# dylkot/cNMF

Measured on AMD Instinct MI355X. Metric: NMF restarts/sec (50000x2000xK5..13), higher is better.
Workload: dtype f32 (exact integer f16 plane x 2 f16 planes with per-row exponent, f32 accumulate)

## Files before the change

cnmf_amd/csrc/gemm_host.hip.h:

```cpp
#pragma once

#include "pass_plan.h"


template <int MTW, int WM, int WN, bool NN, int TBK = BK>
static hipError_t launch_gemm_t(hipStream_t st, const float* A, int lda, const float* B, int ldb,
                                float* C, int ldc, long long cstride, int KC, int Ktot, int J,
                                int nsplit)
{
    constexpr int MW = WM * MTW * 32, JW = WN * 32;
    const int Kper = round_up((Ktot + nsplit - 1) / nsplit, BK);
    dim3 grid((J + JW - 1) / JW, KC / MW, nsplit);
    constexpr size_t lds = gemm_lds_bytes<MTW, WM, WN, NN, TBK>();
    {
        if (hipError_t e_ = dyn_lds_optin((const void*)gemm_kernel<MTW, WM, WN, NN, TBK>, (int)lds)) return e_;
    }
    gemm_kernel<MTW, WM, WN, NN, TBK><<<grid, 256, lds, st>>>(A, lda, B, ldb, C, ldc, cstride, Kper,
                                                             Ktot, J);
    return hipGetLastError();
}

template <bool NN>
static hipError_t launch_gemm(hipStream_t st, int variant, const float* A, int lda, const float* B,
                              int ldb, float* C, int ldc, long long cstride, int KC, int Ktot,
// ... 192 lines not shown
    const int N = (int)ctx->N, G = (int)ctx->G, Np = ctx->N_pad, Gp = ctx->G_pad;
    const size_t pb = (size_t)Np * Gp * 2;
    const size_t fa = (size_t)(Np / G3C_JW) * ((Gp / 16 + 31) / 32) * sizeof(unsigned), fb = (size_t)(Gp / G3C_JW) * ((Np / 16 + 31) / 32) * sizeof(unsigned);
    DevPool pool;
    int* shA = pool.get<int>(Np);
    int* shB = pool.get<int>(Gp);
    POOL_TRY(ctx, pool);
    OwnedLocal<GeneralPlanesF> L;
    HIP_TRY(ctx, hipMalloc(&L.X2h, pb));
    HIP_TRY(ctx, hipMalloc(&L.X2m, pb));
    HIP_TRY(ctx, hipMalloc(&L.Xt2h, pb));
    HIP_TRY(ctx, hipMalloc(&L.Xt2m, pb));
    HIP_TRY(ctx, hipMalloc(&L.sA, (size_t)Np * sizeof(float)));
    HIP_TRY(ctx, hipMalloc(&L.sB, (size_t)Gp * sizeof(float)));
    HIP_TRY(ctx, hipMalloc(&L.onesA, fa));
    HIP_TRY(ctx, hipMalloc(&L.onesB, fb));
    HIP_TRY(ctx, hipMemsetAsync(L.onesA, 0xff, fa, st));
    HIP_TRY(ctx, hipMemsetAsync(L.onesB, 0xff, fb, st));
    x2h_rowshift_kernel<<<(Np + 3) / 4, 256, 0, st>>>(ctx->X, Gp, N, G, 0, Np, shA, L.sA);
    x2h_rowshift_kernel<<<(Gp + 255) / 256, 256, 0, st>>>(ctx->X, Gp, N, G, 1, Gp, shB, L.sB);
    const long long total = (long long)Np * (Gp / 16);
    x2h_planes_kernel<<<(unsigned)((total + 255) / 256), 256, 0, st>>>(ctx->X, Gp, N, G, Np, Gp, G3C_JW, shA,
                                                                        (unsigned short*)L.X2h, (unsigned short*)L.X2m);
    x2h_planes_transpose_kernel<<<dim3(Np / 16, (Gp + 255) / 256), 256, 0, st>>>(ctx->X, Gp, N, G, Gp, Np, G3C_JW, shB,
                                                                                (unsigned short*)L.Xt2h, (unsigned short*)L.Xt2m);
    HIP_TRY(ctx, hipGetLastError());
    HIP_TRY(ctx, hipStreamSynchronize(st));
    ctx->x2.take(L);
    return CNMF_OK;
}

static hipError_t launch_gemm3c(hipStream_t st, const unsigned char* A3, const unsigned char* B1,
                                const unsigned char* Bhi, const unsigned int* hiflag, int Kb,
                                float* C, int ldc, long long cstride, int KC, int Jpad, int nsplit)
{
    {
        if (hipError_t e_ = dyn_lds_optin((const void*)gemm3c_kernel, g3c_lds_bytes(true))) return e_;
    }
    const int kb_per = (Kb + nsplit - 1) / nsplit;
    dim3 grid(Jpad / G3C_JW, KC / G3_MW, (Kb + kb_per - 1) / kb_per);
    gemm3c_kernel<<<grid, 512, g3c_lds_bytes(Bhi != nullptr), st>>>(A3, B1, Bhi, hiflag, Kb, C, ldc, cstride, kb_per);
    return hipGetLastError();
}

static hipError_t launch_gemm3c_streamk(hipStream_t st, const StreamK3& sk, const unsigned char* A3,
                                        const unsigned char* B1, const unsigned char* Bhi,
                                        const unsigned int* hiflag, float* C0, float* C1, float* C2, int ldc)
{
    {
        if (hipError_t e_ = dyn_lds_optin((const void*)gemm3c_streamk_kernel, g3c_lds_bytes(true))) return e_;
    }
    gemm3c_streamk_kernel<<<sk.P, 512, g3c_lds_bytes(Bhi != nullptr), st>>>(A3, B1, Bhi, hiflag, sk.Kb, C0, C1, C2, ldc,
                                                                            sk.MG, sk.T);
    return hipGetLastError();
}


struct G2Launch {
    const unsigned char* A2 = nullptr;
    const float* rscale = nullptr;
    XOperand x{};
    int Kb = 0;
    float* C[3] = {nullptr, nullptr, nullptr};
    int ldc = 0;
    unsigned long long livemask = ~0ull;
    long long cstride = 0; int KC = 0, Jpad = 0, nsplit = 1;
    const StreamK3* sk = nullptr;
    const CdKnobs* kn = nullptr;
};
using G2Fn = hipError_t (*)(hipStream_t, const G2Launch&);
struct G2Entry { G2Form form; G2Fn fn; };

template <int NSUB, bool HI, int VAR = 0, bool PART = false, bool GEN = false>
static hipError_t launch_gemm2h_t(hipStream_t st, const G2Launch& g)
{
    constexpr int lds = g2_lds_bytes(NSUB, HI);
    {
        if (hipError_t e_ = dyn_lds_optin((const void*)gemm2h_kernel<NSUB, HI, VAR, PART, GEN>, lds)) return e_;
    }
    int kb_per = (g.Kb + g.nsplit - 1) / g.nsplit;
    kb_per = ((kb_per + NSUB - 1) / NSUB) * NSUB;
    dim3 grid(g.Jpad / G3C_JW, g.KC / G3_MW, (g.Kb + kb_per - 1) / kb_per);
    gemm2h_kernel<NSUB, HI, VAR, PART, GEN><<<grid, 512, lds, st>>>(g.A2, g.x.plane, HI ? g.x.hi : nullptr, HI ? g.x.flags : nullptr, g.rscale,
                                                                   g.Kb, g.C[0], g.ldc, g.cstride, kb_per, g.x.colscale,
                                                                   PART ? g.livemask : ~0ull);
    return hipGetLastError();
}

template <int NSUB, bool HI, int VAR = 0, bool NTB = true, bool PART = false, bool GEN = false>
static hipError_t launch_gemm2h_streamk_t(hipStream_t st, const G2Launch& g)
{
    constexpr int lds = g2_lds_bytes(NSUB, HI);
    {
        if (hipError_t e_ = dyn_lds_optin((const void*)gemm2h_streamk_kernel<NSUB, HI, VAR, NTB, PART, GEN>, lds)) return e_;
    }
    const int xmap = g2_xmap(G2Form{true, NSUB, HI, VAR, NTB, PART, GEN}, g.kn->g2_xmap);
    gemm2h_streamk_kernel<NSUB, HI, VAR, NTB, PART, GEN><<<g.sk->P, 512, lds, st>>>(g.A2, g.x.plane, HI ? g.x.hi : nullptr,
                                                                                    HI ? g.x.flags : nullptr, g.rscale, g.Kb, g.C[0], g.C[1],
                                                                                    g.C[2], g.ldc, g.sk->MG, g.sk->T, xmap, g.x.colscale,
                                                                                    PART ? g.livemask : ~0ull);
    return hipGetLastError();
}

template <int NSUB, bool HI, int VAR, bool PART, bool GEN>
static constexpr G2Entry g2_ksplit() { return {G2Form{true, NSUB, HI, VAR, false, PART, GEN}, launch_gemm2h_t<NSUB, HI, VAR, PART, GEN>}; }
template <int NSUB, bool HI, int VAR, bool NTB, bool PART, bool GEN>
static constexpr G2Entry g2_streamk() { return {G2Form{true, NSUB, HI, VAR, NTB, PART, GEN}, launch_gemm2h_streamk_t<NSUB, HI, VAR, NTB, PART, GEN>}; }

static constexpr G2Entry G2_KSPLIT[] = {
    g2_ksplit<1, true, 0, false, true>(),  g2_ksplit<1, true, 0, true, true>(),  g2_ksplit<1, true, 4, false, true>(),
    g2_ksplit<1, true, 4, true, true>(),   g2_ksplit<1, true, 0, false, false>(), g2_ksplit<1, true, 0, true, false>(),
    g2_ksplit<2, false, 4, false, false>(), g2_ksplit<2, false, 4, true, false>(), g2_ksplit<1, false, 4, false, false>()};
static constexpr G2Entry G2_STREAMK[] = {
    g2_streamk<1, true, 0, false, true, true>(),   g2_streamk<1, true, 0, false, false, true>(),  g2_streamk<1, true, 0, true, false, true>(),
    g2_streamk<1, true, 4, false, true, true>(),   g2_streamk<1, true, 4, false, false, true>(),  g2_streamk<1, true, 4, true, false, true>(),
    g2_streamk<1, true, 0, false, true, false>(),  g2_streamk<1, true, 0, false, false, false>(), g2_streamk<1, true, 0, true, false, false>(),
    g2_streamk<2, false, 4, false, true, false>(), g2_streamk<2, false, 4, false, false, false>(), g2_streamk<2, false, 4, true, false, false>(),
    g2_streamk<1, false, 4, false, false, false>(), g2_streamk<1, false, 4, true, false, false>()};

static G2Form g2_form_of(const G2Launch& g, int KC, bool shared)
{
    const unsigned long long full = g2_full_mask(KC);
    return g2_form(g.x.hi != nullptr, g.x.colscale != nullptr, g.kn->g2_gen4, g.kn->g2_gvar, gemm2h_nsub(false, g.Kb, g.kn->g2_nsub),
                   (g.livemask & full) != full, shared);
}

static hipError_t launch_gemm2h(hipStream_t st, const G2Launch& g)
{
    G2Form f = g2_form_of(g, g.KC, false);
    f.NTB = false;
    for (const G2Entry& e : G2_KSPLIT) if (e.form == f) return e.fn(st, g);
    return hipErrorInvalidValue;
}

static hipError_t launch_gemm2h_streamk(hipStream_t st, const G2Launch& g)
{
    const G2Form f = g2_form_of(g, g.sk->MG * G3_MW, g.sk->MG > 1);
    for (const G2Entry& e : G2_STREAMK) if (e.form == f) return e.fn(st, g);
    return hipErrorInvalidValue;
}

static hipError_t launch_split2h(hipStream_t st, const float* src, int ld, int rows, int K, unsigned char* dst, int TR,
                                 const double* kscale, const float* rmax_part, int parts, float* inv_scale)
{
    if (split2h_wide(K)) {
        dim3 grid(split2h_col_groups(K, rows), rows / 16);
        split2h_tiled_kernel<16, 16><<<grid, 256, 0, st>>>(src, ld, K, TR, (unsigned short*)dst, kscale, rmax_part, parts, inv_scale);
    } else {
        dim3 grid(split2h_col_groups(K, rows), rows / 64);
        split2h_tiled_kernel<64, 4><<<grid, 256, 0, st>>>(src, ld, K, TR, (unsigned short*)dst, kscale, rmax_part, parts, inv_scale);
    }
    return hipGetLastError();
}

static hipError_t launch_rowmax_part(hipStream_t st, const float* V, int ld, int L, int rows, int span,
                                     const double* kscale, int parts, float* rmax_part)
{
    dim3 grid(parts, rows / 4);
    rowmax_part_kernel<<<grid, 256, 0, st>>>(V, ld, L, span, kscale, parts, rmax_part);
    return hipGetLastError();
}

static int ensure_counts(cnmf_ctx* ctx)
{
    const int fmt = ctx->knobs.gemm3 == 4 ? 4 : 3;
    if (ctx->counts.state == 1 && ctx->counts.fmt != fmt) {
        hipStreamSynchronize(ctx->stream);
        ctx->counts.release();
    }
    if (ctx->counts.state != 0) return CNMF_OK;
    auto absent = [ctx] { ctx->counts.state = -1; return CNMF_OK; };
    const int N = (int)ctx->N, G = (int)ctx->G;
    if (ctx->N_pad % G3C_JW || ctx->G_pad % G3C_JW || ctx->knobs.no_counts || !ctx->count_detect) return absent();
    hipStream_t st = ctx->stream;
    const int chunks = (N + CNT_ROWS - 1) / CNT_ROWS;
    DevPool pool;
    float* part = pool.get<float>((size_t)chunks * G);
    float* vmin = pool.get<float>(G);
    unsigned* fail = pool.get<unsigned>(G, true, st);
    float* unit = pool.get<float>(G);
    double* psx = pool.get<double>((size_t)chunks * G);
    double* psn = pool.get<double>((size_t)chunks * G);
// ... 91 lines not shown
```

cnmf_amd/csrc/kernels_gemm2h.hip.h:

```cpp
#pragma once
#include <hip/hip_runtime.h>
#include "kernels_gemm3.hip.h"

namespace cnmf {

typedef _Float16 f16x8 __attribute__((ext_vector_type(8)));
typedef float f32x4_g __attribute__((ext_vector_type(4)));
#ifdef CNMF_G2_LDS_STORE
constexpr bool G2_LDS_STORE = true;
#else
constexpr bool G2_LDS_STORE = false;
#endif

constexpr int G2_ROWB = 64;
constexpr int G2_A = G3_MW * G2_ROWB;
constexpr int G2_B = G3C_JW * 32;
constexpr float G2_COUNT_BASE = 2048.0f;

constexpr int g2_imgs(int nsub) { return nsub == 1 ? 4 : 3; }
constexpr int g2_img_bytes(int nsub, bool with_hi) { return nsub * (G2_A + (with_hi ? 2 : 1) * G2_B); }
constexpr int g2_lds_bytes(int nsub, bool with_hi) { return g2_imgs(nsub) * g2_img_bytes(nsub, with_hi); }

__device__ __forceinline__ unsigned short f16_bits(float x)
{
    const _Float16 h = (_Float16)x;
    return __builtin_bit_cast(unsigned short, h);
}
__device__ __forceinline__ float f16_to_f32(unsigned short b) { return (float)__builtin_bit_cast(_Float16, b); }

__device__ __forceinline__ int g2_row_shift(float mx)
{
    if (!(mx > 0.f)) return 0;
    int e;
    frexpf(mx, &e);
    const int s = 15 - e;
    return s > 120 ? 120 : (s < -110 ? -110 : s);
}

__device__ __forceinline__ void split2h(float y, unsigned short& h, unsigned short& m)
{
    h = f16_bits(y);
    m = f16_bits(y - f16_to_f32(h));
}

struct SplitFused { const int* shift_in; int* shift_out; };
template <int TROWS, int TKB>
__device__ __forceinline__ void split2h_tiled_body(const float* __restrict__ src, int ld, int K, int TR,
                                                   unsigned short* __restrict__ dst, const double* __restrict__ kscale,
                                                   const float* __restrict__ rmax_part, int parts,
                                                   float* __restrict__ inv_scale, int bx, int nbx, int by,
                                                   unsigned short* tile_, float* red_, SplitFused fu = SplitFused{nullptr, nullptr})
{
    static_assert(TROWS * TKB == 256, "tile = 256 (row, block) pairs");
    constexpr int NQ = 256 / TROWS;
    constexpr int KQ = TKB * 4;
    constexpr int RPP = 256 / KQ;
    unsigned short (*tile)[TROWS][32] = reinterpret_cast<unsigned short (*)[TROWS][32]>(tile_);
    float (*red)[TROWS] = reinterpret_cast<float (*)[TROWS]>(red_);
    const int t = threadIdx.x;
    const int r0 = by * TROWS;
    const int kq = t % KQ, rr = t / KQ;
    const int ntiles = K / (16 * TKB);
    const bool fused = fu.shift_in != nullptr;
    float4 v[4];
    if (!fused) {
        const int k0 = bx * 16 * TKB;
#pragma unroll
        for (int i = 0; i < 4; ++i)
            v[i] = *reinterpret_cast<const float4*>(src + (size_t)(r0 + rr + RPP * i) * ld + k0 + kq * 4);
    }
    {
        const int row = t % TROWS, qt = t / TROWS;
        float mx = 0.f;
        for (int p0 = qt; p0 < parts; p0 += 8 * NQ) {
            float v[8];
#pragma unroll
            for (int j = 0; j < 8; ++j) v[j] = (p0 + j * NQ < parts) ? rmax_part[(size_t)(r0 + row) * parts + p0 + j * NQ] : 0.f;
#pragma unroll
            for (int j = 0; j < 8; ++j) mx = fmaxf(mx, v[j]);
        }
        red[qt][row] = mx;
    }
    __syncthreads();
    int sh[4];
    bool redo = false;
#pragma unroll
    for (int i = 0; i < 4; ++i) {
        const int row = rr + RPP * i;
        float mx = 0.f;
#pragma unroll
        for (int q = 0; q < NQ; ++q) mx = fmaxf(mx, red[q][row]);
        sh[i] = g2_row_shift(mx);
        if (fused) {
            const int su = fu.shift_in[r0 + row];
            const float ymax = ldexpf(mx, su);
            const bool ok = !(mx > 0.f) || (ymax < 60000.0f && ymax >= 1024.0f);
            const bool keep = !(mx > 0.f) || (ymax < 46340.0f && ymax >= 8192.0f);
            if (bx == 0 && kq == 0) fu.shift_out[r0 + row] = (ok && keep) ? su : sh[i];
            if (ok) sh[i] = su; else redo = true;
        }
        if (bx == 0 && kq == 0) inv_scale[r0 + row] = ldexpf(1.0f, -sh[i]);
    }
    if (fused) {
        if (!__syncthreads_or(redo ? 1 : 0)) return;
// ... 164 lines not shown
{
    if (!transpose) {
        const int row = blockIdx.x * 4 + (threadIdx.x >> 6), lane = threadIdx.x & 63;
        if (row >= rows_pad) return;
        float mx = 0.f;
        if (row < N) for (int g = lane; g < G; g += 64) mx = fmaxf(mx, X[(size_t)row * ld + g]);
#pragma unroll
        for (int o = 32; o > 0; o >>= 1) mx = fmaxf(mx, __shfl_xor(mx, o, 64));
        if (lane == 0) { const int s = g2_row_shift(mx); shift[row] = s; inv_scale[row] = ldexpf(1.0f, -s); }
    } else {
        const int g = blockIdx.x * 256 + threadIdx.x;
        if (g >= rows_pad) return;
        float mx = 0.f;
        if (g < G) for (int r = 0; r < N; ++r) mx = fmaxf(mx, X[(size_t)r * ld + g]);
        const int s = g2_row_shift(mx);
        shift[g] = s; inv_scale[g] = ldexpf(1.0f, -s);
    }
}

__global__ __launch_bounds__(256) void x2h_planes_kernel(const float* __restrict__ X, int ld, int N, int G, int rows_pad,
                                                         int K, int TR, const int* __restrict__ shift,
                                                         unsigned short* __restrict__ dst_h, unsigned short* __restrict__ dst_m)
{
    const long long t = (long long)blockIdx.x * 256 + threadIdx.x;
    const int Kb = K / 16;
    if (t >= (long long)rows_pad * Kb) return;
    const int row = (int)(t / Kb), kb = (int)(t % Kb);
    const int s = shift[row];
    unsigned short ph[16], pm[16];
#pragma unroll
    for (int i = 0; i < 16; ++i) {
        const int g = kb * 16 + i;
        const float x = (row < N && g < G) ? X[(size_t)row * ld + g] : 0.f;
        split2h(ldexpf(x, s), ph[i], pm[i]);
    }
    const size_t blk = (size_t)(row / TR) * Kb + kb;
    store_plane_row_swz(dst_h + (blk * TR + (row % TR)) * 16, ph, row % TR);
    store_plane_row_swz(dst_m + (blk * TR + (row % TR)) * 16, pm, row % TR);
}

__global__ __launch_bounds__(256) void x2h_planes_transpose_kernel(const float* __restrict__ X, int ld, int N, int G,
                                                                   int rows_pad, int K, int TR,
                                                                   const int* __restrict__ shift,
                                                                   unsigned short* __restrict__ dst_h,
                                                                   unsigned short* __restrict__ dst_m)
{
    const int j = blockIdx.y * 256 + threadIdx.x;
    const int kb = blockIdx.x;
    if (j >= rows_pad) return;
    const int Kb = K / 16;
    const int s = shift[j];
    unsigned short ph[16], pm[16];
#pragma unroll
    for (int i = 0; i < 16; ++i) {
        const int c = kb * 16 + i;
        const float x = (j < G && c < N) ? X[(size_t)c * ld + j] : 0.f;
        split2h(ldexpf(x, s), ph[i], pm[i]);
    }
    const size_t blk = (size_t)(j / TR) * Kb + kb;
    store_plane_row_swz(dst_h + (blk * TR + (j % TR)) * 16, ph, j % TR);
    store_plane_row_swz(dst_m + (blk * TR + (j % TR)) * 16, pm, j % TR);
}

__global__ __launch_bounds__(256) void count_max_base_kernel(const float* __restrict__ X, int ld, int N, int G,
                                                             const float* __restrict__ unit, float base,
                                                             unsigned* __restrict__ any_big)
{
    const int g = blockIdx.x * 256 + threadIdx.x;
    if (g >= G) return;
    const float u = unit[g];
    if (u <= 0.f) return;
    const int r0 = blockIdx.y * 256, r1 = min(N, r0 + 256);
    bool big = false;
    for (int r = r0; r < r1; ++r) big |= rintf(X[(size_t)r * ld + g] / u) > base;
    if (big) atomicOr(any_big, 1u);
}

struct G2NoEpi { static constexpr bool enabled = false; };
template <int NSUB, bool HI, int VAR = 0, bool NTB = true, bool PART = false, bool GEN = false, class EPI = G2NoEpi>
__device__ __forceinline__ void gemm2h_segment(const unsigned char* __restrict__ A2, const unsigned char* __restrict__ B1,
                                               const unsigned char* __restrict__ Bhi,
                                               const unsigned int* __restrict__ hiflag,
                                               const float* __restrict__ rscale,
                                               int Kb, float* __restrict__ C, int ldc, int m0, int j0, int kb0,
                                               int nkb, unsigned char* smem, const float* __restrict__ cscale = nullptr,
                                               unsigned live = 0xffu, const EPI* epi = nullptr, bool whole_tile = false)
{
    constexpr int IMGS = g2_imgs(NSUB);
    constexpr int IMG = g2_img_bytes(NSUB, HI);
    constexpr int OFF_B = NSUB * G2_A;
    constexpr int OFF_H = OFF_B + NSUB * G2_B;
    constexpr int NA = NSUB * 2, NB = NSUB;
    constexpr int NDMA = NA + NB;
    const int tid = threadIdx.x;
    const int lane = tid & 63, wave = tid >> 6;
    const int grp = wave >> 2, wn = wave & 3;
    const int li = lane & 31, h = lane >> 5;
    const int nst = nkb / NSUB;
    const unsigned lv = PART ? (unsigned)__builtin_amdgcn_readfirstlane((int)((live >> (grp * 4)) & 0xfu)) : 0xfu;
#define G2_LIVE(m_) (!PART || ((lv >> (m_)) & 1u))

    const size_t jblk = ((size_t)(j0 / G3C_JW) * Kb + kb0);
    const unsigned char* abase = A2 + ((size_t)(m0 / G3_MW) * Kb + kb0) * G2_A + tid * 16;
    const unsigned char* bbase = B1 + jblk * G2_B + tid * 16;
    const unsigned char* hbase = HI ? Bhi + jblk * G2_B + tid * 16 : nullptr;
    unsigned int fw[5] = {0u, 0u, 0u, 0u, 0u};
    if (HI) {
        const int KW = (Kb + 31) >> 5, w0 = kb0 >> 5;
        const unsigned int* fr = hiflag + (size_t)(j0 / G3C_JW) * KW;
#pragma unroll
        for (int w = 0; w < 5; ++w)
            fw[w] = (nkb > 129) ? 0xFFFFFFFFu : ((w0 + w < KW) ? __builtin_amdgcn_readfirstlane(fr[w0 + w]) : 0u);
    }
    const int fbit0 = kb0 & 31;

    f32x16_3 acc[4][2];
#pragma unroll
    for (int m = 0; m < 4; ++m)
#pragma unroll
        for (int n = 0; n < 2; ++n)
#pragma unroll
            for (int r = 0; r < 16; ++r) acc[m][n][r] = 0.f;

    const int a_row = (grp * 128 + li) * G2_ROWB;
    const int a_s0 = ((0 + h) ^ ((li >> 2) & 3)) * 16, a_s1 = ((2 + h) ^ ((li >> 2) & 3)) * 16;
    const int b_off = OFF_B + (wn * 64 + li) * 32 + (h ^ ((li >> 3) & 1)) * 16;

#define G2_BLKFLAG(b_) (HI && ((fw[(fbit0 + (b_)) >> 5 > 4 ? 4 : (fbit0 + (b_)) >> 5] >> ((fbit0 + (b_)) & 31)) & 1u))
#define G2_ISSUE(s_)                                                                               \
    {                                                                                              \
        unsigned char* d_ = smem + ((s_) % IMGS) * IMG + wave * 1024;                              \
        const unsigned char* a_ = abase + (size_t)(s_) * (NSUB * G2_A);                            \
        _Pragma("unroll") for (int i = 0; i < NA; ++i)                                             \
            __builtin_amdgcn_global_load_lds(G3_AS1(a_ + i * 8192), G3_AS3(d_ + i * 8192), 16, 0, 0); \
                                        \
        _Pragma("unroll") for (int i = 0; i < NB; ++i)                                             \
            __builtin_amdgcn_global_load_lds(G3_AS1(bbase + (size_t)(s_) * (NSUB * G2_B) + i * 8192), \
                                             G3_AS3(d_ + OFF_B + i * 8192), 16, 0, NTB ? 2 : 0);   \
        if (HI) {                                                                                  \
            _Pragma("unroll") for (int i = 0; i < NB; ++i)                                         \
                if (G2_BLKFLAG((s_) * NSUB + i))                                                   \
                    __builtin_amdgcn_global_load_lds(G3_AS1(hbase + (size_t)(s_) * (NSUB * G2_B) + i * 8192), \
                                                     G3_AS3(d_ + OFF_H + i * 8192), 16, 0, NTB ? 2 : 0); \
        }                                                                                          \
    }
#define G2_FRAG(ptr_) __builtin_bit_cast(f16x8, *reinterpret_cast<const u32x4*>(ptr_))
#define G2_READ(s_)                                                                                \
    {                                                                                              \
        const unsigned char* bb = smem + ((s_) % IMGS) * IMG;                                      \
        _Pragma("unroll") for (int u = 0; u < NSUB; ++u) {                                         \
            _Pragma("unroll") for (int n = 0; n < 2; ++n) bq[u][n] = G2_FRAG(bb + b_off + u * G2_B + n * 32 * 32); \
            if (HI) { _Pragma("unroll") for (int n = 0; n < 2; ++n)                                \
                          bh[u][n] = G2_FRAG(bb + b_off + NSUB * G2_B + u * G2_B + n * 32 * 32); } \
            _Pragma("unroll") for (int m = 0; m < 4; ++m) {                                        \
                aq[u][m][0] = G2_FRAG(bb + u * G2_A + a_row + m * 32 * G2_ROWB + a_s0);            \
                aq[u][m][1] = G2_FRAG(bb + u * G2_A + a_row + m * 32 * G2_ROWB + a_s1);            \
            }                                                                                      \
        }                                                                                          \
        __builtin_amdgcn_sched_barrier(0);                                                         \
    }
#define G2_MFMA(b_, u_, m_, q_)                                                                    \
    if (G2_LIVE(m_)) {                                                                             \
    acc[m_][0] = __builtin_amdgcn_mfma_f32_32x32x16_f16(aq[u_][m_][q_], b_[u_][0], acc[m_][0], 0, 0, 0); \
    acc[m_][1] = __builtin_amdgcn_mfma_f32_32x32x16_f16(aq[u_][m_][q_], b_[u_][1], acc[m_][1], 0, 0, 0); }
#define G2_MFMA4(b_, u_, ma_, mb_)                                                                 \
    G2_MFMA(b_, u_, ma_, 1) G2_MFMA(b_, u_, mb_, 1) G2_MFMA(b_, u_, ma_, 0) G2_MFMA(b_, u_, mb_, 0)
#define G2_MFMA2H(b_, u_, ma_, mb_) G2_MFMA(b_, u_, ma_, 0) G2_MFMA(b_, u_, mb_, 0)
#define G2_HALF(ma_, mb_)                                                                          \
    _Pragma("unroll") for (int u = 0; u < NSUB; ++u) {                                             \
        G2_MFMA4(bq, u, ma_, mb_)                                                                  \
        if (HI) { if (hi_blk[u]) { if constexpr (GEN) { G2_MFMA2H(bh, u, ma_, mb_) } else { G2_MFMA4(bh, u, ma_, mb_) } } } \
    }
#define G2_WAIT_AHEAD(cnt_)                                                                        \
    {                                                                                              \
        if constexpr ((cnt_) * NDMA == 0) G3_WAIT_VM(0);                                           \
        else if constexpr ((cnt_) * NDMA == 3) G3_WAIT_VM(3);                                      \
        else if constexpr ((cnt_) * NDMA == 6) G3_WAIT_VM(6);                                      \
        else if constexpr ((cnt_) * NDMA == 12) G3_WAIT_VM(12);                                    \
        else G3_WAIT_VM(0);                                                                        \
    }

    f16x8 bq[NSUB][2], bh[NSUB][2], aq[NSUB][4][2];
    constexpr int AHEAD = IMGS - 1;
    constexpr bool SPREAD = VAR >= 1 && NSUB == 2 && !HI;
    constexpr bool SPREADG = VAR >= 1 && NSUB == 1 && ((HI && GEN) || !HI);
    constexpr bool PRIO = false;
    constexpr bool NOMFMA = VAR == 2, NODMA = VAR == 3 || VAR == 6 || VAR == 7, SPLITRD = VAR >= 4;
    static_assert(VAR != 1 && VAR != 5, "instruction streams 1 and 5 were retired");
    constexpr bool NOREAD = VAR == 6 || VAR == 7;
    constexpr bool NOBAR = VAR == 7;
    G3_WAIT_VM(0);
    G2_ISSUE(0)
    if (nst > 1) G2_ISSUE(1)
    if (AHEAD > 2 && nst > 2) G2_ISSUE(2)
    if (AHEAD > 2 && nst > 2) G2_WAIT_AHEAD(2) else if (nst > 1) G2_WAIT_AHEAD(1) else G2_WAIT_AHEAD(0)
    if (grp == 1) G3_RAW_BARRIER()
    if constexpr (SPREADG) {
        static_assert(!SPREADG || (IMGS == 4 && NA == 2 && NB == 1), "one-block spread stream: four images, pieces A0 A1 B (Bhi)");
#define G2G_PIECE(s_, i_)                                                                          \
        {                                                                                          \
            unsigned char* d_ = smem + ((s_) % IMGS) * IMG + wave * 1024;                          \
            if ((i_) < NA)                                                                         \
                __builtin_amdgcn_global_load_lds(G3_AS1(abase + (size_t)(s_) * G2_A + (i_) * 8192), \
                                                 G3_AS3(d_ + (i_) * 8192), 16, 0, 0);              \
            else if ((i_) == NA)                                                                   \
                __builtin_amdgcn_global_load_lds(G3_AS1(bbase + (size_t)(s_) * G2_B), G3_AS3(d_ + OFF_B), 16, 0, NTB ? 2 : 0); \
            else if constexpr (HI)                                                                 \
                __builtin_amdgcn_global_load_lds(G3_AS1(hbase + (size_t)(s_) * G2_B), G3_AS3(d_ + OFF_H), 16, 0, NTB ? 2 : 0); \
            __builtin_amdgcn_sched_barrier(0);                                                     \
        }
#define G2G_READ_A(s_)                                                                             \
        {                                                                                          \
            const unsigned char* bb = smem + ((s_) % IMGS) * IMG;                                  \
            _Pragma("unroll") for (int n = 0; n < 2; ++n) bq[0][n] = G2_FRAG(bb + b_off + n * 32 * 32); \
            _Pragma("unroll") for (int m = 0; m < 2; ++m) {                                        \
                aq[0][m][1] = G2_FRAG(bb + a_row + m * 32 * G2_ROWB + a_s1);                       \
                aq[0][m][0] = G2_FRAG(bb + a_row + m * 32 * G2_ROWB + a_s0);                       \
            }                                                                                      \
            if constexpr (HI) { _Pragma("unroll") for (int n = 0; n < 2; ++n) bh[0][n] = G2_FRAG(bb + b_off + G2_B + n * 32 * 32); } \
            __builtin_amdgcn_sched_barrier(0);                                                     \
        }
#define G2G_READ_B(s_)                                                                             \
        {                                                                                          \
            const unsigned char* bb = smem + ((s_) % IMGS) * IMG;                                  \
            _Pragma("unroll") for (int m = 2; m < 4; ++m) {                                        \
                aq[0][m][1] = G2_FRAG(bb + a_row + m * 32 * G2_ROWB + a_s1);                       \
                aq[0][m][0] = G2_FRAG(bb + a_row + m * 32 * G2_ROWB + a_s0);                       \
            }                                                                                      \
            __builtin_amdgcn_sched_barrier(0);                                                     \
        }
#define G2G_STEP(MORE_)                                                                            \
        {                                                                                          \
            G3_RAW_BARRIER()                                         \
            G2G_READ_A(s)                                                                          \
            G2_MFMA(bq, 0, 0, 1) G2_MFMA(bq, 0, 1, 1)                                              \
            if (MORE_) G2G_PIECE(s + AHEAD, 0)                                                     \
            G2_MFMA(bq, 0, 0, 0) G2_MFMA(bq, 0, 1, 0)                                              \
            G2G_READ_B(s)                                                                          \
            if (MORE_) G2G_PIECE(s + AHEAD, 1)                                                     \
            if constexpr (HI) { G2_MFMA(bh, 0, 0, 0) G2_MFMA(bh, 0, 1, 0) }                        \
            asm volatile("s_waitcnt lgkmcnt(0)" ::: "memory");                                     \
             \
            if (s + 1 < nst) { if (MORE_) { if constexpr (HI) G3_WAIT_VM(6); else G3_WAIT_VM(5); } else G3_WAIT_VM(0); } \
            G3_RAW_BARRIER()                                                              \
            G2_MFMA(bq, 0, 2, 1) G2_MFMA(bq, 0, 3, 1)                                              \
            if (MORE_) G2G_PIECE(s + AHEAD, 2)                                                     \
            G2_MFMA(bq, 0, 2, 0) G2_MFMA(bq, 0, 3, 0)                                              \
            if constexpr (HI) { if (MORE_) G2G_PIECE(s + AHEAD, 3)                                 \
                                G2_MFMA(bh, 0, 2, 0) G2_MFMA(bh, 0, 3, 0) }                        \
        }
        {
            int s = 0;
            const int n_main = nst - AHEAD;
            for (; s < n_main; ++s) G2G_STEP(true)
            for (; s < nst; ++s) G2G_STEP(false)
        }
#undef G2G_STEP
#undef G2G_READ_B
#undef G2G_READ_A
#undef G2G_PIECE
    } else if constexpr (!SPREAD) {
        for (int s = 0; s < nst; ++s) {
            bool hi_blk[NSUB];
#pragma unroll
            for (int u = 0; u < NSUB; ++u) hi_blk[u] = G2_BLKFLAG(s * NSUB + u);
            G3_RAW_BARRIER()
            if (s + AHEAD < nst) G2_ISSUE(s + AHEAD)
            G2_READ(s)
            if (PRIO) __builtin_amdgcn_s_setprio(1);
            G2_HALF(0, 1)
            if (PRIO) __builtin_amdgcn_s_setprio(0);
            asm volatile("s_waitcnt lgkmcnt(0)" ::: "memory");
            if (s + 1 < nst) {
                if (AHEAD > 2 && s + 3 < nst) G2_WAIT_AHEAD(2) else if (s + 2 < nst) G2_WAIT_AHEAD(1) else G2_WAIT_AHEAD(0)
// ... 12 lines not shown
                                                 G3_AS3(d_ + (i_) * 8192), 16, 0, 0);              \
            else                                                                                   \
                __builtin_amdgcn_global_load_lds(G3_AS1(bbase + (size_t)(s_) * (NSUB * G2_B) + ((i_) - NA) * 8192), \
                                                 G3_AS3(d_ + OFF_B + ((i_) - NA) * 8192), 16, 0, NTB ? 2 : 0); \
            __builtin_amdgcn_sched_barrier(0);                                                     \
        }
#define G2_MF(u_, m_, q_)                                                                          \
        if constexpr (NOMFMA) { asm volatile("" :: "v"(aq[u_][m_][q_]), "v"(bq[u_][0]), "v"(bq[u_][1])); }        \
        else { G2_MFMA(bq, u_, m_, q_) }
#define G2_READ_A(s_)                                                                              \
    {                                                                                              \
        const unsigned char* bb = smem + ((s_) % IMGS) * IMG;                                      \
        _Pragma("unroll") for (int u = 0; u < NSUB; ++u) {                                         \
            _Pragma("unroll") for (int n = 0; n < 2; ++n) bq[u][n] = G2_FRAG(bb + b_off + u * G2_B + n * 32 * 32); \
            _Pragma("unroll") for (int m = 0; m < 2; ++m) {                                        \
                aq[u][m][1] = G2_FRAG(bb + u * G2_A + a_row + m * 32 * G2_ROWB + a_s1);            \
                aq[u][m][0] = G2_FRAG(bb + u * G2_A + a_row + m * 32 * G2_ROWB + a_s0);            \
            }                                                                                      \
        }                                                                                          \
        __builtin_amdgcn_sched_barrier(0);                                                         \
    }
#define G2_READ_B(s_)                                                                              \
    {                                                                                              \
        const unsigned char* bb = smem + ((s_) % IMGS) * IMG;                                      \
        _Pragma("unroll") for (int u = 0; u < NSUB; ++u)                                           \
            _Pragma("unroll") for (int m = 2; m < 4; ++m) {                                        \
                aq[u][m][1] = G2_FRAG(bb + u * G2_A + a_row + m * 32 * G2_ROWB + a_s1);            \
                aq[u][m][0] = G2_FRAG(bb + u * G2_A + a_row + m * 32 * G2_ROWB + a_s0);            \
            }                                                                                      \
        __builtin_amdgcn_sched_barrier(0);                                                         \
    }
#define G2_STEP(MORE_)                                                                             \
        {                                                                                          \
            if constexpr (!NOBAR) G3_RAW_BARRIER()                                        \
            if constexpr (NOREAD) { if (s == 0) { G2_READ(s) } }                                   \
            else if constexpr (SPLITRD) { G2_READ_A(s) } else { G2_READ(s) }                       \
            G2_MF(0, 0, 1) G2_MF(0, 1, 1)                                                          \
            if (MORE_) G2_PIECE(s + AHEAD, 0)                                                      \
            G2_MF(0, 0, 0) G2_MF(0, 1, 0)                                                          \
            if constexpr (SPLITRD && !NOREAD) { G2_READ_B(s) }                                     \
            if (MORE_) G2_PIECE(s + AHEAD, 1)                                                      \
            G2_MF(1, 0, 1) G2_MF(1, 1, 1)                                                          \
            if (MORE_) G2_PIECE(s + AHEAD, 2)                                                      \
            G2_MF(1, 0, 0) G2_MF(1, 1, 0)                                                          \
            asm volatile("s_waitcnt lgkmcnt(0)" ::: "memory");                                     \
             \
            if (s + 1 < nst) { if (MORE_) G3_WAIT_VM(3); else G3_WAIT_VM(0); }                     \
            if constexpr (!NOBAR) G3_RAW_BARRIER()                                        \
            G2_MF(0, 2, 1) G2_MF(0, 3, 1)                                                          \
            if (MORE_) G2_PIECE(s + AHEAD, 3)                                                      \
            G2_MF(0, 2, 0) G2_MF(0, 3, 0)                                                          \
            if (MORE_) G2_PIECE(s + AHEAD, 4)                                                      \
            G2_MF(1, 2, 1) G2_MF(1, 3, 1)                                                          \
            if (MORE_) G2_PIECE(s + AHEAD, 5)                                                      \
            G2_MF(1, 2, 0) G2_MF(1, 3, 0)                                                          \
        }
        {
            int s = 0;
            const int n_main = NODMA ? 0 : nst - AHEAD;
            for (; s < n_main; ++s) G2_STEP(true)
            for (; s < nst; ++s) G2_STEP(false)
        }
#undef G2_STEP
#undef G2_READ_B
#undef G2_READ_A
#undef G2_MF
#undef G2_PIECE
    }
    if (grp == 0) G3_RAW_BARRIER()
#undef G2_WAIT_AHEAD
#undef G2_HALF
#undef G2_MFMA2H
#undef G2_MFMA4
#undef G2_MFMA
#undef G2_READ
#undef G2_FRAG
#undef G2_ISSUE
#undef G2_BLKFLAG

    if constexpr (EPI::enabled) {
        if (whole_tile && epi->on) { (*epi)(acc, rscale, C, ldc, m0, j0, smem); return; }
    }
    if (C == nullptr) return;
    const int j = j0 + wn * 64 + li;
    const float cs[2] = {(HI && cscale) ? cscale[j] : 1.0f, (HI && cscale) ? cscale[j + 32] : 1.0f};
    if constexpr (!PART && G2_LDS_STORE && g2_lds_bytes(NSUB, HI) >= 8 * 16384) {
        float* tw = reinterpret_cast<float*>(smem) + wave * 4096;
#pragma unroll
        for (int mp = 0; mp < 2; ++mp) {
#pragma unroll
            for (int mm = 0; mm < 2; ++mm) {
                const int m = 2 * mp + mm;
#pragma unroll
                for (int n = 0; n < 2; ++n)
#pragma unroll
                    for (int r = 0; r < 16; ++r) {
                        const int rl = 4 * h + (r & 3) + 8 * (r >> 2);
                        tw[(mm * 32 + rl) * 64 + n * 32 + li] = (acc[m][n][r] * rscale[m0 + grp * 128 + m * 32 + rl]) * cs[n];
                    }
            }
            __builtin_amdgcn_wave_barrier();
#pragma unroll
            for (int i = 0; i < 16; ++i) {
                const int c = 4 * i + (lane >> 4);
                const f32x4_g v = *reinterpret_cast<const f32x4_g*>(tw + c * 64 + 4 * (lane & 15));
                *reinterpret_cast<f32x4_g*>(C + (size_t)(m0 + grp * 128 + mp * 64 + c) * ldc + j0 + wn * 64 + 4 * (lane & 15)) = v;
            }
            __builtin_amdgcn_wave_barrier();
        }
    } else {
#pragma unroll
    for (int m = 0; m < 4; ++m) {
        if (!G2_LIVE(m)) continue;
        const int cbase = m0 + grp * 128 + m * 32 + 4 * h;
#pragma unroll
        for (int n = 0; n < 2; ++n)
#pragma unroll
            for (int r = 0; r < 16; ++r) {
                const int row = cbase + (r & 3) + 8 * (r >> 2);
                C[(size_t)row * ldc + j + n * 32] = (acc[m][n][r] * rscale[row]) * cs[n];
            }
    }
    }
#undef G2_LIVE
}

template <int NSUB, bool HI, int VAR = 0, bool PART = false, bool GEN = false>
__global__ __launch_bounds__(512) void gemm2h_kernel(const unsigned char* __restrict__ A2,
                                                     const unsigned char* __restrict__ B1,
                                                     const unsigned char* __restrict__ Bhi,
                                                     const unsigned int* __restrict__ hiflag,
                                                     const float* __restrict__ rscale, int Kb,
                                                     float* __restrict__ C, int ldc, long long c_split_stride,
                                                     int kb_per, const float* __restrict__ cscale = nullptr,
                                                     unsigned long long livemask = ~0ull)
{
    extern __shared__ __attribute__((aligned(16))) unsigned char smem3[];
    int jt = blockIdx.x, mg = blockIdx.y, z = blockIdx.z;
    if ((gridDim.z & 7) == 0) {
        const int L = blockIdx.x + (int)gridDim.x * (blockIdx.y + (int)gridDim.y * blockIdx.z);
        const int xcd = L & 7, idx = L >> 3;
        jt = idx % (int)gridDim.x;
        mg = (idx / (int)gridDim.x) % (int)gridDim.y;
        z = xcd + 8 * (idx / (int)(gridDim.x * gridDim.y));
    }
    const int kb0 = z * kb_per;
    const int nkb = min(kb_per, Kb - kb0);
    gemm2h_segment<NSUB, HI, VAR, true, PART, GEN>(A2, B1, Bhi, hiflag, rscale, Kb, C ? C + (size_t)z * c_split_stride : nullptr, ldc, mg * G3_MW,
                                              jt * G3C_JW, kb0, nkb, smem3, cscale, (unsigned)((livemask >> (8 * mg)) & 0xffu));
}

template <int NSUB, bool HI, int VAR = 0, bool NTB = true, bool PART = false, bool GEN = false, class EPI = G2NoEpi>
__global__ __launch_bounds__(512) void gemm2h_streamk_kernel(const unsigned char* __restrict__ A2,
                                                             const unsigned char* __restrict__ B1,
                                                             const unsigned char* __restrict__ Bhi,
                                                             const unsigned int* __restrict__ hiflag,
                                                             const float* __restrict__ rscale, int Kb,
                                                             float* __restrict__ C0, float* __restrict__ C1,
                                                             float* __restrict__ C2, int ldc, int MG, int T, int xmap,
                                                             const float* __restrict__ cscale = nullptr,
                                                             unsigned long long livemask = ~0ull, EPI epi = EPI{})
{
    extern __shared__ __attribute__((aligned(16))) unsigned char smem3[];
    const int Ks = Kb / NSUB;
    const long long U = (long long)T * Ks;
    const int P = (int)gridDim.x;
    const int q = (xmap && MG > 1 && P % MG == 0) ? ((int)blockIdx.x % MG) * (P / MG) + (int)blockIdx.x / MG : (int)blockIdx.x;
    long long u = U * q / P;
    const long long u1 = U * (q + 1) / P;
    const int NJ = T / MG;
    while (u < u1) {
        const int tile = (int)(u / Ks), ks = (int)(u % Ks);
        const int ke = (int)min((long long)Ks, ks + (u1 - u));
        const int mg = tile / NJ, jt = tile % NJ;
        gemm2h_segment<NSUB, HI, VAR, NTB, PART, GEN, EPI>(A2, B1, Bhi, hiflag, rscale, Kb, (ks == 0) ? C0 : (ke == Ks ? C1 : C2), ldc, mg * G3_MW,
                                                 jt * G3C_JW, ks * NSUB, (ke - ks) * NSUB, smem3, cscale,
                                                 (unsigned)((livemask >> (8 * mg)) & 0xffu), &epi, ks == 0 && ke == Ks);
        u += ke - ks;
        G3_WAIT_VM(0);
        __syncthreads();
    }
}

}
```

cnmf_amd/csrc/pass_plan.h:

```cpp
#pragma once

#include <algorithm>
#include <cstdint>
#include <vector>

constexpr int PLAN_BK = 32, PLAN_G3_MW = 256, PLAN_G3_JW = 128, PLAN_G3C_JW = 256, PLAN_G3_BK = 16, PLAN_KSMALL = 64;

struct PadShape { int N_pad, G_pad; };

static inline int plan_round_up(int64_t v, int m) { return (int)(((v + m - 1) / m) * m); }

static inline int sweep_chunks(int parts_knob, int L) { const int64_t m = 256ll * parts_knob; return std::max(1, (int)(((int64_t)L + m - 1) / m)); }
static inline int sweep_parts(int parts_knob, int L) { const int c = sweep_chunks(parts_knob, L); return (L + 256 * c - 1) / (256 * c); }

enum class SweepForm { W, W_A64, W_PLN, W_PLN_A64, H_RMX, H_PSUM, INVALID };

static inline bool sweep_a64(int ldv) { return 64ll * ldv * 4 > 0x7fffffffll; }

static inline SweepForm sweep_form(bool has_planes_out, bool psum, bool exact_rmax, bool a64, int tiers = 7)
{
    if (has_planes_out) {
        if (psum || exact_rmax || (tiers & 8)) return SweepForm::INVALID;
        return a64 ? SweepForm::W_PLN_A64 : SweepForm::W_PLN;
    }
    if (psum) return (tiers & 8) ? SweepForm::INVALID : SweepForm::H_PSUM;
    if (exact_rmax) return SweepForm::H_RMX;
    return a64 ? SweepForm::W_A64 : SweepForm::W;
}

static inline int pick_nsplit(PadShape s, int KC)
{
    const int jt = (s.G_pad + 127) / 128;
    const int mg = std::max(1, KC / 128);
    int n = std::max(1, 512 / (jt * mg));
    const int max_by_k = std::max(1, s.N_pad / 256);
    return std::min(n, max_by_k);
}

static inline int effective_splits(int Ktot, int nsplit)
{
    const int Kper = plan_round_up((Ktot + nsplit - 1) / nsplit, PLAN_BK);
    return (Ktot + Kper - 1) / Kper;
}

static inline int pick_nsplit_A(PadShape s, int KC)
{
    const int T = (s.N_pad / 128) * std::max(1, KC / 128);
    if (T > 256) return 1;
    int n = std::max(1, 512 / T);
    n = std::min(n, std::max(1, s.G_pad / (4 * PLAN_BK)));
    return effective_splits(s.G_pad, std::min(n, 16));
}

static inline int gemm3_wg_slots(int gemm3, int wg_slots_knob)
{
    if (wg_slots_knob >= 32 && gemm3 >= 2) return wg_slots_knob;
    return gemm3 >= 2 ? 256 : 512;
}

static inline int pick_nsplit_A3(PadShape s, int KC, int jw, int wg_slots)
{
    const int T = std::max(1, s.N_pad / jw) * std::max(1, KC / PLAN_G3_MW);
    const int Kb = s.G_pad / PLAN_G3_BK;
    int n = std::max(1, std::min(wg_slots / T, Kb / 8));
    const int kb_per = (Kb + n - 1) / n;
    return (Kb + kb_per - 1) / kb_per;
}

static inline int pick_nsplit3(PadShape s, int KC, int jw, int wg_slots)
{
    const int tiles = std::max(1, s.G_pad / jw) * std::max(1, KC / PLAN_G3_MW);
    const int Kb = s.N_pad / PLAN_G3_BK;
    int n = std::max(1, std::min(wg_slots / std::max(1, tiles), Kb / 16));
    const int kb_per = (Kb + n - 1) / n;
    return (Kb + kb_per - 1) / kb_per;
}

struct SplitCaps { int nsplit, nsplitA; };
static inline SplitCaps size_splits(PadShape s, int KC, bool use3, int wg_slots)
{
    SplitCaps c{pick_nsplit(s, KC), pick_nsplit_A(s, KC)};
    if (use3) {
        c.nsplit = std::max(c.nsplit, std::max(pick_nsplit3(s, KC, PLAN_G3_JW, wg_slots), pick_nsplit3(s, KC, PLAN_G3C_JW, wg_slots)));
        c.nsplitA = std::max(c.nsplitA, std::max(pick_nsplit_A3(s, KC, PLAN_G3_JW, wg_slots), pick_nsplit_A3(s, KC, PLAN_G3C_JW, wg_slots)));
    }
    return c;
}

struct StreamK {
    bool on = false;
    int MG = 1, T = 0, nk = 0, P = 0, mw = 128;
    std::vector<unsigned char> split;
};

static inline StreamK plan_streamk(int KC, PadShape s, int n_wg_slots, bool no_streamk)
{
    StreamK sk;
    if (KC % 128 != 0 || no_streamk) return sk;
    sk.MG = KC / sk.mw;
    sk.T = sk.MG * (s.N_pad / 128);
// ... 120 lines not shown
```

Before: 218.6.

## Prefetch row/col scales into LDS and use buffer stores in gemm2h epilogue

Row and column scale factors are loaded asynchronously into a new LDS region via global_load_lds at kernel start, replacing per-element global loads of rscale and cscale in the epilogue. The C store path switches to raw buffer stores with a scalar row offset when addresses fit in 32 bits, and falls back to plain stores otherwise. The unused LDS-staged store variant is removed. LDS footprint grows by 1-2 KB per block, which may affect occupancy.

```diff
diff --git a/cnmf_amd/csrc/gemm_host.hip.h b/cnmf_amd/csrc/gemm_host.hip.h
--- a/cnmf_amd/csrc/gemm_host.hip.h
+++ b/cnmf_amd/csrc/gemm_host.hip.h
@@ -298,7 +298,7 @@
     kb_per = ((kb_per + NSUB - 1) / NSUB) * NSUB;
     dim3 grid(g.Jpad / G3C_JW, g.KC / G3_MW, (g.Kb + kb_per - 1) / kb_per);
     gemm2h_kernel<NSUB, HI, VAR, PART, GEN><<<grid, 512, lds, st>>>(g.A2, g.x.plane, HI ? g.x.hi : nullptr, HI ? g.x.flags : nullptr, g.rscale,
-                                                                   g.Kb, g.C[0], g.ldc, g.cstride, kb_per, g.x.colscale,
+                                                                   g.Kb, g.C[0], g.ldc, g2_store_a64(g.ldc) ? 1 : 0, g.cstride, kb_per, g.x.colscale,
                                                                    PART ? g.livemask : ~0ull);
     return hipGetLastError();
 }
@@ -313,7 +313,7 @@
     const int xmap = g2_xmap(G2Form{true, NSUB, HI, VAR, NTB, PART, GEN}, g.kn->g2_xmap);
     gemm2h_streamk_kernel<NSUB, HI, VAR, NTB, PART, GEN><<<g.sk->P, 512, lds, st>>>(g.A2, g.x.plane, HI ? g.x.hi : nullptr,
                                                                                     HI ? g.x.flags : nullptr, g.rscale, g.Kb, g.C[0], g.C[1],
-                                                                                    g.C[2], g.ldc, g.sk->MG, g.sk->T, xmap, g.x.colscale,
+                                                                                    g.C[2], g.ldc, g2_store_a64(g.ldc) ? 1 : 0, g.sk->MG, g.sk->T, xmap, g.x.colscale,
                                                                                     PART ? g.livemask : ~0ull);
     return hipGetLastError();
 }
diff --git a/cnmf_amd/csrc/kernels_gemm2h.hip.h b/cnmf_amd/csrc/kernels_gemm2h.hip.h
--- a/cnmf_amd/csrc/kernels_gemm2h.hip.h
+++ b/cnmf_amd/csrc/kernels_gemm2h.hip.h
@@ -6,11 +6,6 @@
 
 typedef _Float16 f16x8 __attribute__((ext_vector_type(8)));
 typedef float f32x4_g __attribute__((ext_vector_type(4)));
-#ifdef CNMF_G2_LDS_STORE
-constexpr bool G2_LDS_STORE = true;
-#else
-constexpr bool G2_LDS_STORE = false;
-#endif
 
 constexpr int G2_ROWB = 64;
 constexpr int G2_A = G3_MW * G2_ROWB;
@@ -19,7 +14,8 @@
 
 constexpr int g2_imgs(int nsub) { return nsub == 1 ? 4 : 3; }
 constexpr int g2_img_bytes(int nsub, bool with_hi) { return nsub * (G2_A + (with_hi ? 2 : 1) * G2_B); }
-constexpr int g2_lds_bytes(int nsub, bool with_hi) { return g2_imgs(nsub) * g2_img_bytes(nsub, with_hi); }
+constexpr int g2_scale_off(int nsub, bool with_hi) { return g2_imgs(nsub) * g2_img_bytes(nsub, with_hi); }
+constexpr int g2_lds_bytes(int nsub, bool with_hi) { return g2_scale_off(nsub, with_hi) + (with_hi ? 2048 : 1024); }
 
 __device__ __forceinline__ unsigned short f16_bits(float x)
 {
@@ -350,7 +346,7 @@
                                                const unsigned char* __restrict__ Bhi,
                                                const unsigned int* __restrict__ hiflag,
                                                const float* __restrict__ rscale,
-                                               int Kb, float* __restrict__ C, int ldc, int m0, int j0, int kb0,
+                                               int Kb, float* __restrict__ C, int ldc, bool a64, int m0, int j0, int kb0,
                                                int nkb, unsigned char* smem, const float* __restrict__ cscale = nullptr,
                                                unsigned live = 0xffu, const EPI* epi = nullptr, bool whole_tile = false)
 {
@@ -458,6 +454,13 @@
     constexpr bool NOREAD = VAR == 6 || VAR == 7;
     constexpr bool NOBAR = VAR == 7;
     G3_WAIT_VM(0);
+    const int wave_e = __builtin_amdgcn_readfirstlane(tid) >> 6;
+    const unsigned char* rs_src = reinterpret_cast<const unsigned char*>(rscale + m0);
+    const unsigned char* cs_src = reinterpret_cast<const unsigned char*>(reinterpret_cast<uintptr_t>(cscale) + (uintptr_t)((long long)(j0 - 256) * 4));
+    asm volatile("" : "+s"(rs_src), "+s"(cs_src));
+    float* sc_lds = reinterpret_cast<float*>(smem + g2_scale_off(NSUB, HI));
+    if (wave == 0) __builtin_amdgcn_global_load_lds(G3_AS1(rs_src + (unsigned)tid * 16u), G3_AS3(sc_lds), 16, 0, 0);
+    if constexpr (HI) { if (cscale && wave == 1) __builtin_amdgcn_global_load_lds(G3_AS1(cs_src + (unsigned)tid * 16u), G3_AS3(sc_lds + 256), 16, 0, 0); }
     G2_ISSUE(0)
     if (nst > 1) G2_ISSUE(1)
     if (AHEAD > 2 && nst > 2) G2_ISSUE(2)
@@ -636,46 +639,54 @@
         if (whole_tile && epi->on) { (*epi)(acc, rscale, C, ldc, m0, j0, smem); return; }
     }
     if (C == nullptr) return;
-    const int j = j0 + wn * 64 + li;
-    const float cs[2] = {(HI && cscale) ? cscale[j] : 1.0f, (HI && cscale) ? cscale[j + 32] : 1.0f};
-    if constexpr (!PART && G2_LDS_STORE && g2_lds_bytes(NSUB, HI) >= 8 * 16384) {
-        float* tw = reinterpret_cast<float*>(smem) + wave * 4096;
-#pragma unroll
-        for (int mp = 0; mp < 2; ++mp) {
-#pragma unroll
-            for (int mm = 0; mm < 2; ++mm) {
-                const int m = 2 * mp + mm;
+    int lane_e;
+    asm volatile("v_mbcnt_lo_u32_b32 %0, -1, 0\n\tv_mbcnt_hi_u32_b32 %0, -1, %0" : "=v"(lane_e));
+    const int li_e = lane_e & 31, h_e = lane_e >> 5, grp_e = wave_e >> 2;
+    const int jl = (wave_e & 3) * 64 + li_e;
+    const float* rs_w = sc_lds + grp_e * 128 + 4 * h_e;
+    f32x4_g s4[4][4];
+#define G2_SCALES(m_)                                                                              \
+    {                                                                                              \
+        _Pragma("unroll") for (int q = 0; q < 4; ++q) s4[m_][q] = *reinterpret_cast<const f32x4_g*>(rs_w + (m_) * 32 + 8 * q); \
+    }
+    G2_SCALES(0)
+    float cs[2] = {1.0f, 1.0f};
+    if (HI && cscale) { cs[0] = sc_lds[256 + jl]; cs[1] = sc_lds[256 + jl + 32]; }
+    if (!a64) {
+        const __amdgpu_buffer_rsrc_t rC = __builtin_amdgcn_make_buffer_rsrc((void*)(C + (size_t)(m0 + grp_e * 128) * ldc), 0,
+                                                                            (int)(128u * (unsigned)ldc * 4u), 0x00020000);
+        const int voff = (j0 + jl + 4 * h_e * ldc) * 4, row_bytes = ldc * 4;
+#pragma unroll
+        for (int m = 0; m < 4; ++m) {
+            if (m < 3) G2_SCALES(m + 1)
+            __builtin_amdgcn_sched_barrier(0);
+            if (!G2_LIVE(m)) continue;
+#pragma unroll
+            for (int q = 0; q < 4; ++q)
 #pragma unroll
                 for (int n = 0; n < 2; ++n)
 #pragma unroll
-                    for (int r = 0; r < 16; ++r) {
-                        const int rl = 4 * h + (r & 3) + 8 * (r >> 2);
-                        tw[(mm * 32 + rl) * 64 + n * 32 + li] = (acc[m][n][r] * rscale[m0 + grp * 128 + m * 32 + rl]) * cs[n];
-                    }
-            }
-            __builtin_amdgcn_wave_barrier();
-#pragma unroll
-            for (int i = 0; i < 16; ++i) {
-                const int c = 4 * i + (lane >> 4);
-                const f32x4_g v = *reinterpret_cast<const f32x4_g*>(tw + c * 64 + 4 * (lane & 15));
-                *reinterpret_cast<f32x4_g*>(C + (size_t)(m0 + grp * 128 + mp * 64 + c) * ldc + j0 + wn * 64 + 4 * (lane & 15)) = v;
-            }
-            __builtin_amdgcn_wave_barrier();
+                    for (int i = 0; i < 4; ++i)
+                        __builtin_amdgcn_raw_buffer_store_b32(__builtin_bit_cast(unsigned, (acc[m][n][4 * q + i] * s4[m][q][i]) * cs[n]), rC,
+                                                              voff + n * 128, (m * 32 + 8 * q + i) * row_bytes, 0);
         }
     } else {
 #pragma unroll
-    for (int m = 0; m < 4; ++m) {
-        if (!G2_LIVE(m)) continue;
-        const int cbase = m0 + grp * 128 + m * 32 + 4 * h;
-#pragma unroll
-        for (int n = 0; n < 2; ++n)
-#pragma unroll
-            for (int r = 0; r < 16; ++r) {
-                const int row = cbase + (r & 3) + 8 * (r >> 2);
-                C[(size_t)row * ldc + j + n * 32] = (acc[m][n][r] * rscale[row]) * cs[n];
-            }
-    }
-    }
+        for (int m = 0; m < 4; ++m) {
+            if (m < 3) G2_SCALES(m + 1)
+            __builtin_amdgcn_sched_barrier(0);
+            if (!G2_LIVE(m)) continue;
+            const int cbase = m0 + grp_e * 128 + m * 32 + 4 * h_e;
+#pragma unroll
+            for (int q = 0; q < 4; ++q)
+#pragma unroll
+                for (int n = 0; n < 2; ++n)
+#pragma unroll
+                    for (int i = 0; i < 4; ++i)
+                        C[(size_t)(cbase + 8 * q + i) * ldc + j0 + jl + n * 32] = (acc[m][n][4 * q + i] * s4[m][q][i]) * cs[n];
+        }
+    }
+#undef G2_SCALES
 #undef G2_LIVE
 }
 
@@ -685,7 +696,7 @@
                                                      const unsigned char* __restrict__ Bhi,
                                                      const unsigned int* __restrict__ hiflag,
                                                      const float* __restrict__ rscale, int Kb,
-                                                     float* __restrict__ C, int ldc, long long c_split_stride,
+                                                     float* __restrict__ C, int ldc, int a64, long long c_split_stride,
                                                      int kb_per, const float* __restrict__ cscale = nullptr,
                                                      unsigned long long livemask = ~0ull)
 {
@@ -700,7 +711,7 @@
     }
     const int kb0 = z * kb_per;
     const int nkb = min(kb_per, Kb - kb0);
-    gemm2h_segment<NSUB, HI, VAR, true, PART, GEN>(A2, B1, Bhi, hiflag, rscale, Kb, C ? C + (size_t)z * c_split_stride : nullptr, ldc, mg * G3_MW,
+    gemm2h_segment<NSUB, HI, VAR, true, PART, GEN>(A2, B1, Bhi, hiflag, rscale, Kb, C ? C + (size_t)z * c_split_stride : nullptr, ldc, a64 != 0, mg * G3_MW,
                                               jt * G3C_JW, kb0, nkb, smem3, cscale, (unsigned)((livemask >> (8 * mg)) & 0xffu));
 }
 
@@ -711,7 +722,7 @@
                                                              const unsigned int* __restrict__ hiflag,
                                                              const float* __restrict__ rscale, int Kb,
                                                              float* __restrict__ C0, float* __restrict__ C1,
-                                                             float* __restrict__ C2, int ldc, int MG, int T, int xmap,
+                                                             float* __restrict__ C2, int ldc, int a64, int MG, int T, int xmap,
                                                              const float* __restrict__ cscale = nullptr,
                                                              unsigned long long livemask = ~0ull, EPI epi = EPI{})
 {
@@ -727,7 +738,7 @@
         const int tile = (int)(u / Ks), ks = (int)(u % Ks);
         const int ke = (int)min((long long)Ks, ks + (u1 - u));
         const int mg = tile / NJ, jt = tile % NJ;
-        gemm2h_segment<NSUB, HI, VAR, NTB, PART, GEN, EPI>(A2, B1, Bhi, hiflag, rscale, Kb, (ks == 0) ? C0 : (ke == Ks ? C1 : C2), ldc, mg * G3_MW,
+        gemm2h_segment<NSUB, HI, VAR, NTB, PART, GEN, EPI>(A2, B1, Bhi, hiflag, rscale, Kb, (ks == 0) ? C0 : (ke == Ks ? C1 : C2), ldc, a64 != 0, mg * G3_MW,
                                                  jt * G3C_JW, ks * NSUB, (ke - ks) * NSUB, smem3, cscale,
                                                  (unsigned)((livemask >> (8 * mg)) & 0xffu), &epi, ks == 0 && ke == Ks);
         u += ke - ks;
diff --git a/cnmf_amd/csrc/pass_plan.h b/cnmf_amd/csrc/pass_plan.h
--- a/cnmf_amd/csrc/pass_plan.h
+++ b/cnmf_amd/csrc/pass_plan.h
@@ -16,6 +16,8 @@
 enum class SweepForm { W, W_A64, W_PLN, W_PLN_A64, H_RMX, H_PSUM, INVALID };
 
 static inline bool sweep_a64(int ldv) { return 64ll * ldv * 4 > 0x7fffffffll; }
+
+static inline bool g2_store_a64(int ldc) { return 256ll * ldc * 4 > 0x7fffffffll; }
 
 static inline SweepForm sweep_form(bool has_planes_out, bool psum, bool exact_rmax, bool a64, int tiers = 7)
 {
```

Result: no change. 219.9 (median of 6 runs) (+0.6%).
